# GregDMeyer/dynamite

Hardware: AMD Instinct MI355X
Metric: matrix-free H|psi> Gamplitudes/s, random-field Heisenberg (higher is better)
Workload: dtype f64 (complex128)

## Files before the change

### dynamite_amd/_lib.py

```python
import ctypes as C
import os

import numpy as np

from . import build as _build

_HERE = os.path.dirname(os.path.abspath(__file__))

i64p = C.POINTER(C.c_int64)
f64p = C.POINTER(C.c_double)
vp = C.c_void_p


class Subspace(C.Structure):
    _fields_ = [("type", C.c_int32), ("L", C.c_int64), ("space", C.c_int64), ("k", C.c_int64),
                ("ld_nchoosek", C.c_int64), ("nchoosek", i64p), ("dim", C.c_int64),
                ("state_map", i64p), ("rmap_indices", i64p), ("rmap_states", i64p), ("vec_swizzle", C.c_int32),
                ("site_perm", C.POINTER(C.c_int8))]


class Partition(C.Structure):
    _fields_ = [("rank", C.c_int32), ("nranks", C.c_int32)]


MULT_FN = C.CFUNCTYPE(C.c_int, vp, vp, vp)
REDUCE_FN = C.CFUNCTYPE(C.c_int, vp, f64p, C.c_int)


class Hooks(C.Structure):
    _fields_ = [("ctx", vp), ("mult", MULT_FN), ("allreduce_sum", REDUCE_FN),
                ("allreduce_max", REDUCE_FN)]


class SolverStats(C.Structure):
    _fields_ = [("reason", C.c_int32), ("its", C.c_int32), ("matvecs", C.c_int32),
                ("nconv", C.c_int32), ("err_est", C.c_double)]


MAXSEG, MAXBSEG, MAXR = 4, 8, 16


LP_COUNT = 9
LP_NAMES = ["tile_real_k0", "tile_real", "tile_cplx", "tile_kvar_real", "tile_kvar_cplx", "gather_real",
            "gather_kvar_real", "gather_cplx", "gather_kvar_cplx"]
LP_KVAR, LP_CPLX, LP_GATHER = (3, 4, 6, 8), (2, 4, 7, 8), (5, 6, 7, 8)


class DevQuad(C.Structure):
    _fields_ = [("mask_tile", C.c_uint32), ("mask_loc", C.c_uint32), ("src", C.c_uint32),
                ("nslots", C.c_uint32), ("sign_tile", C.c_uint32 * 4), ("sign_ext", C.c_uint64 * 4),
                ("coeff", C.c_double * 4)]


class DevPass(C.Structure):
    _fields_ = [("nseg", C.c_int32), ("seg_off", C.c_int32 * MAXSEG), ("seg_len", C.c_int32 * MAXSEG),
                ("seg_pos", C.c_int32 * MAXSEG), ("nbseg", C.c_int32), ("bseg_off", C.c_int32 * MAXBSEG),
                ("bseg_len", C.c_int32 * MAXBSEG), ("bseg_pos", C.c_int32 * MAXBSEG),
                ("sign_base", C.c_uint64), ("accumulate", C.c_int32), ("need_tile", C.c_int32),
                ("has_diag", C.c_int32), ("cache_policy", C.c_int32), ("dext_begin", C.c_uint32), ("dext_end", C.c_uint32),
                ("dbucket", C.c_uint32 * (MAXR + 1)), ("loop", C.c_uint32 * (LP_COUNT + 1)),
                ("nquads", C.c_int32), ("n_eff", C.c_int32), ("quads", vp), ("dot_out", vp), ("zinit", vp), ("zscale", C.c_double), ("zinit2", vp), ("z2re", C.c_double), ("z2im", C.c_double),
                ("tile_bits", C.c_int32), ("log_rows", C.c_int32),
                ("swz_shift", C.c_int32), ("swz_xor_y", C.c_uint32), ("swz_xor_src", C.c_uint32), ("block_offset", C.c_uint32),
                ("pos_tmask", C.c_uint32), ("dtile", vp), ("tabs", vp), ("tabvals", vp), ("tab_loop", C.c_uint32 * 3),
                ("pad_tab", C.c_uint32), ("gbucket", C.c_uint32 * (MAXR + 1)), ("pad_g", C.c_uint32)]


class DevTab(C.Structure):
    _fields_ = [("mask_tile", C.c_uint32), ("mask_loc", C.c_uint32), ("src", C.c_uint32), ("first", C.c_uint32),
                ("z_tile", C.c_uint32), ("flags", C.c_uint32), ("tpos", C.c_uint32), ("twid", C.c_uint32),
                ("epos", C.c_uint32), ("ewid", C.c_uint32), ("z_ext", C.c_uint64), ("ik", C.c_uint64),
                ("ksign", C.c_uint32), ("nbits", C.c_uint32)]


class Xfer(C.Structure):
    _fields_ = [("partner", C.c_int32), ("pass_id", C.c_int32), ("offset", C.c_int64), ("count", C.c_int64)]


MAT_DEFAULT, MAT_FORCE_GATHER, MAT_USE_GLDS, MAT_HOST_ONLY = 0, 1, 2, 4
MAT_REAL_PACKED = 16
EXCHANGE_AUTO, EXCHANGE_PARTNER, EXCHANGE_TRANSPOSE = 0, 1, 2
PHASE_ALL, PHASE_EXCHANGE, PHASE_COMPUTE = 0, 1, 2
MAT_AMIN_SHIFT = 8
WHICH = {"lowest": 0, "highest": 1, "exterior": 2, "target": 3}
CONVERGED_TOL, CONVERGED_ITS, DIVERGED_ITS, DIVERGED_BREAKDOWN, DIVERGED_SYMMETRY_LOST = 1, 2, -1, -2, -3

SIGNATURES = {
    "dnm_last_error": (C.c_char_p, []),
    "dnm_version": (C.c_int, []),
    "dnm_device_count": (C.c_int, [C.POINTER(C.c_int)]),
    "dnm_set_device": (C.c_int, [C.c_int]),
    "dnm_malloc": (C.c_int, [C.POINTER(vp), C.c_size_t]),
    "dnm_free": (C.c_int, [vp]),
    "dnm_memcpy_h2d": (C.c_int, [vp, vp, C.c_size_t, vp]),
    "dnm_memcpy_d2h": (C.c_int, [vp, vp, C.c_size_t, vp]),
    "dnm_stream_synchronize": (C.c_int, [vp]),
    "dnm_subspace_dim": (C.c_int, [C.POINTER(Subspace), i64p]),
    "dnm_idx_to_state": (C.c_int, [C.POINTER(Subspace), C.c_int64, i64p, i64p]),
    "dnm_state_to_idx": (C.c_int, [C.POINTER(Subspace), C.c_int64, i64p, i64p]),
    "dnm_mat_create": (C.c_int, [C.c_int64, i64p, i64p, i64p, f64p, C.POINTER(Subspace),
                                 C.POINTER(Subspace), C.c_int, C.c_int, C.POINTER(Partition),
                                 C.POINTER(vp)]),
    "dnm_check_conserves": (C.c_int, [C.c_int64, i64p, i64p, i64p, f64p, C.POINTER(Subspace),
                                      C.POINTER(Subspace), C.c_int, C.POINTER(C.c_int), vp]),
    "dnm_reduced_density_matrix": (C.c_int, [vp, C.POINTER(Subspace), C.c_int, i64p, vp, vp]),
    "dnm_vec_set_random_swz": (C.c_int, [vp, C.c_int64, C.c_uint64, C.c_int64, C.c_int, vp]),
    "dnm_vec_swizzle_copy": (C.c_int, [vp, vp, C.c_int64, C.c_int, vp]),
    "dnm_vec_unpack_real": (C.c_int, [vp, vp, C.c_int64, C.c_int, C.c_int, vp]),
    "dnm_vec_layout_unpack_real": (C.c_int, [C.POINTER(Subspace), C.POINTER(Partition), vp, vp, vp]),
    "dnm_vec_layout_size": (C.c_int, [C.POINTER(Subspace), C.POINTER(C.c_int64)]),
    "dnm_vec_layout_partition": (C.c_int, [C.POINTER(Subspace), C.c_int, C.c_int, i64p, i64p, i64p, i64p]),
    "dnm_vec_layout_blocks": (C.c_int, [C.POINTER(Subspace), C.c_int64, i64p, i64p, i64p]),
    "dnm_vec_layout_copy": (C.c_int, [C.POINTER(Subspace), C.POINTER(Partition), vp, vp, C.c_int, vp]),
    "dnm_vec_layout_copy_f64": (C.c_int, [C.POINTER(Subspace), C.POINTER(Partition), vp, vp, C.c_int, vp]),
    "dnm_vec_layout_zero_padding": (C.c_int, [C.POINTER(Subspace), C.POINTER(Partition), vp, vp]),
    "dnm_vec_layout_positions": (C.c_int, [C.POINTER(Subspace), C.POINTER(Partition), C.c_int64, vp, vp, vp]),
    "dnm_vec_layout_positions_host": (C.c_int, [C.POINTER(Subspace), C.POINTER(Partition), C.c_int64, i64p, i64p]),
    "dnm_vec_layout_set_random": (C.c_int, [C.POINTER(Subspace), C.POINTER(Partition), vp, C.c_uint64, vp]),
# ... 122 lines not shown
```

### dynamite_amd/csrc/mat.cpp

```cpp
#include "mat.h"
#include "vec_api.h"
#include "row_fused.h"

#include <algorithm>
#include <cstring>

namespace dnm {

static thread_local std::string g_err;

void set_error(const char *fmt, ...) {
  char buf[1024];
  va_list ap;
  va_start(ap, fmt);
  vsnprintf(buf, sizeof(buf), fmt, ap);
  va_end(ap);
  g_err = buf;
}

int DevBuf::alloc(size_t nbytes) {
  release();
  if (nbytes == 0) nbytes = 16;
  DNM_HIP(hipMalloc(&p, nbytes));
  bytes = nbytes;
// ... 377 lines not shown
            auto it = std::find_if(all.begin(), all.end(), [&](const auto &g) { return g.first == st; });
            if (it == all.end()) { all.push_back({st, {}}); it = all.end() - 1; }
            it->second.push_back(t);
          }
        std::stable_sort(all.begin(), all.end(), [](const auto &a, const auto &b) { return a.second.size() > b.second.size(); });
        for (auto &g : all)
          if (g.second.size() >= 3 && groups.size() < MAXDGROUPS) groups.push_back(std::move(g));
      }
      auto grouped = [&](uint32_t st) {
        return std::any_of(groups.begin(), groups.end(), [&](const auto &g) { return g.first == st; });
      };
      for (int j = 0; j < R; ++j) {
        lst.clear();
        for (const RowTerm &t : dm->terms) {
          uint32_t st = compress_to_tile(t.sign & tb, ps);
          if (st == 0 || (int)(st >> lognt) != j) continue;
          if (use_table && (t.sign & ~tb) == 0) {
            for (uint32_t tc = 0; tc < (1u << B); ++tc)
              out->h_dtile[tc] += (__builtin_popcount(tc & st) & 1) ? -t.coeff : t.coeff;
          } else if ((t.sign & ~tb) != 0 && grouped(st)) {
            continue;
          } else {
            lst.push_back(t);
          }
        }
        d.dbucket[j] = (uint32_t)quads.size();
        push_diag_list(lst);
      }
      for (int j = R; j <= MAXR; ++j) d.dbucket[j] = (uint32_t)quads.size();
      std::vector<std::pair<uint32_t, uint32_t>> where(groups.size());
      for (size_t g = 0; g < groups.size(); ++g) {
        std::vector<RowTerm> outside = groups[g].second;
        for (RowTerm &t : outside) t.sign &= ~tb;
        where[g].first = (uint32_t)quads.size();
        push_diag_list(outside);
        where[g].second = (uint32_t)quads.size() - where[g].first;
      }
      for (int j = 0; j < R; ++j) {
        d.gbucket[j] = (uint32_t)quads.size();
        for (size_t g = 0; g < groups.size(); ++g) {
          if ((int)(groups[g].first >> lognt) != j) continue;
          DevQuad q = empty_quad();
          q.sign_tile[0] = groups[g].first;
          q.mask_loc = where[g].first;
          q.src = where[g].second;
          q.nslots = 1;
          quads.push_back(q);
        }
      }
      for (int j = R; j <= MAXR; ++j) d.gbucket[j] = (uint32_t)quads.size();
    }
  }

  struct Rec { int loop; DevQuad q; };
  std::vector<Rec> recs;
  std::vector<DevTab> tabs_tile, tabs_gather;
  std::vector<double> tabvals;
  auto push_tabs = [&](const RowMask &m, uint64_t mloc, bool gather, int src) -> bool {
    std::vector<uint64_t> zs;
    if (!table_form(op, m, &zs)) return false;
    const int nb = __builtin_popcountll(m.mask);
    int pb[MAXTABBITS];
    for (int q = 0, pos = 0; pos < 64; ++pos)
      if ((m.mask >> pos) & 1ull) pb[q++] = pos;
    for (uint64_t z : zs) {
      DevTab T;
      memset(&T, 0, sizeof(T));
      T.mask_tile = compress_to_tile(mloc & tb, ps);
      T.mask_loc = (uint32_t)mloc;
      T.src = (uint32_t)src;
      T.nbits = (uint32_t)nb;
      const uint32_t zt = compress_to_tile(z & tb, ps);
      T.z_tile = zt & ((1u << lognt) - 1u);
      T.z_ext = z & ~tb;
      T.first = (uint32_t)(tabvals.size() / 2);
      for (int k = 0; k < R; ++k)
        if (__builtin_popcount((uint32_t)k & (zt >> lognt)) & 1) T.ksign |= 1u << k;
      for (int q = 0; q < nb; ++q) {
        if ((tb >> pb[q]) & 1ull) {
          const int tpos = __builtin_ctz(compress_to_tile((uint64_t)1 << pb[q], ps));
          if (tpos < lognt) {
            T.tpos |= (uint32_t)tpos << (8 * q);
            T.twid |= 1u << (8 * q);
          } else {
            T.flags |= 1u;
            for (int k = 0; k < R; ++k)
              if ((k >> (tpos - lognt)) & 1) T.ik |= (uint64_t)1 << (4 * k + q);
          }
        } else {
          T.epos |= (uint32_t)pb[q] << (8 * q);
          T.ewid |= 1u << (8 * q);
        }
      }
      for (int j = 0; j < (1 << nb); ++j) {
        uint64_t rowbits = 0;
        for (int q = 0; q < nb; ++q)
          if ((j >> q) & 1) rowbits |= (uint64_t)1 << pb[q];
        double re = 0.0, im = 0.0;
        for (const RowTerm &t : m.terms) {
          if ((t.sign & ~m.mask) != z) continue;
          const double c = (__builtin_popcountll(rowbits & t.sign & m.mask) & 1) ? -t.coeff : t.coeff;
          (t.is_imag ? im : re) += c;
        }
        tabvals.push_back(re);
        tabvals.push_back(im);
      }
      if (z == zs.back()) T.flags |= 2u;
      (gather ? tabs_gather : tabs_tile).push_back(T);
    }
    return true;
  };
  auto push_mask = [&](int idx, bool gather, int src) {
    const RowMask &m = op.masks[idx];
    const uint64_t mloc = m.mask & (((uint64_t)1 << n_eff) - 1);
    if (!gather) DNM_CHECK((mloc & ~tb) == 0, "internal: tile mask leaves the tile");
    if (push_tabs(m, mloc, gather, src)) return 0;
    std::vector<const RowTerm *> re, im;
    for (const RowTerm &t : m.terms) (t.is_imag ? im : re).push_back(&t);
    size_t ir = 0, ii = 0;
    while (ir < re.size() || ii < im.size()) {
      DevQuad q = empty_quad();
      q.mask_tile = compress_to_tile(mloc & tb, ps);
      q.mask_loc = (uint32_t)mloc;
      q.src = (uint32_t)src;
      q.nslots = m.pack_flip ? 1u : 0u;
      bool kvar = false, cplx = false;
      for (int s = 0; s < 2 && ir < re.size(); ++s, ++ir) {
        set_slot(q, s, *re[ir]);
        kvar |= (q.sign_tile[s] >> lognt) != 0;
      }
      for (int s = 2; s < 4 && ii < im.size(); ++s, ++ii) {
        set_slot(q, s, *im[ii]);
        kvar |= (q.sign_tile[s] >> lognt) != 0;
        cplx = true;
      }
      int loop;
      if (gather) loop = kvar ? (cplx ? LP_GATHER_KVAR_CPLX : LP_GATHER_KVAR_REAL) : (cplx ? LP_GATHER_CPLX : LP_GATHER_REAL);
      else if (kvar) loop = cplx ? LP_TILE_KVAR_CPLX : LP_TILE_KVAR_REAL;
      else if (cplx) loop = LP_TILE_CPLX;
      else loop = (q.mask_tile >> lognt) == 0 ? LP_TILE_REAL_K0 : LP_TILE_REAL;
      recs.push_back({loop, q});
    }
    return 0;
  };
  for (int idx : ps.tile_masks) DNM_TRY(push_mask(idx, false, 0));
  for (size_t i = 0; i < ps.gather_masks.size(); ++i)
    DNM_TRY(push_mask(ps.gather_masks[i], true, ps.gather_src[i]));
  for (int lp = 0; lp < LP_COUNT; ++lp) {
    d.loop[lp] = (uint32_t)quads.size();
    for (const Rec &r : recs) if (r.loop == lp) quads.push_back(r.q);
  }
  d.loop[LP_COUNT] = (uint32_t)quads.size();

  d.nquads = (int32_t)quads.size();
  d.need_tile = (d.has_diag || !ps.tile_masks.empty()) ? 1 : 0;
  d.tab_loop[0] = 0;
  d.tab_loop[1] = (uint32_t)tabs_tile.size();
  d.tab_loop[2] = (uint32_t)(tabs_tile.size() + tabs_gather.size());
  out->h_tabs = tabs_tile;
  out->h_tabs.insert(out->h_tabs.end(), tabs_gather.begin(), tabs_gather.end());
  out->h_tabvals = tabvals;
  d.tabs = nullptr;
  d.tabvals = nullptr;
  if (!out->h_tabs.empty() && !A.host_only) {
    DNM_TRY(out->tabs.upload(out->h_tabs.data(), out->h_tabs.size() * sizeof(DevTab)));
    DNM_TRY(out->tabvals.upload(out->h_tabvals.data(), out->h_tabvals.size() * sizeof(double)));
    d.tabs = (const DevTab *)out->tabs.p;
    d.tabvals = (const double *)out->tabvals.p;
  }
  out->h_quads = quads;
  if (!A.host_only) DNM_TRY(out->quads.upload(quads.data(), quads.size() * sizeof(DevQuad)));
  d.quads = (const DevQuad *)out->quads.p;
  d.dtile = nullptr;
  if (!out->h_dtile.empty() && !A.host_only) {
    DNM_TRY(out->dtile.upload(out->h_dtile.data(), out->h_dtile.size() * sizeof(double)));
    d.dtile = (const double *)out->dtile.p;
  }
  out->partner = ps.partner;
  out->n_eff = n_eff;
  out->y_off = ps.y_off;
  out->src_off = ps.src_off;
  return 0;
}

static hipStream_t S(void *stream) { return (hipStream_t)stream; }

static int launch_pass(const dnm_mat *A, const PassOnDevice &p, const DevPass &d, const void *x, void *y,
                       const void *xr, hipStream_t st, unsigned nparts = 1) {
  return launch_tile_pass(d, d.tile_bits, d.log_rows, (A->flags & DNM_MAT_USE_GLDS) != 0, p.n_eff, x, y, xr, st, nparts);
}

static size_t pass_dot_partials(const dnm_mat *, const PassOnDevice &p) {
  return (size_t)1 << (p.n_eff - p.desc.tile_bits);
}

}

using namespace dnm;

namespace dnm {
std::vector<ScMask> sc_masks(const std::vector<int64_t> &masks, const std::vector<int64_t> &mask_offsets,
                             const std::vector<int64_t> &signs, const std::vector<double> &rcoef, int L, bool xparity) {
  std::vector<ScMask> scm(masks.size());
// ... 1086 lines not shown
int dnm_mat_exchange_plan(const dnm_mat *A, int *nsend, dnm_xfer *sends, int *nrecv, dnm_xfer *recvs) {
  DNM_CHECK(A && nsend && nrecv, "null argument");
  *nsend = (int)A->plan.sends.size();
  *nrecv = (int)A->remote_passes.size();
  if (sends)
    for (size_t i = 0; i < A->plan.sends.size(); ++i)
      sends[i] = {A->plan.sends[i].partner, -1, A->plan.sends[i].offset, A->plan.sends[i].count};
  if (recvs)
    for (size_t i = 0; i < A->remote_passes.size(); ++i) {
      const auto &p = A->remote_passes[i];
      recvs[i] = {p->partner, (int32_t)i, p->src_off, (int64_t)1 << p->n_eff};
    }
  return 0;
}

int dnm_mat_mult_remote(dnm_mat *A, int32_t recv_index, const void *x_recv, void *y, void *stream) {
  DNM_CHECK(A && x_recv && y, "null argument");
  DNM_CHECK(!A->host_only, "host-only handle cannot multiply");
  DNM_CHECK(recv_index >= 0 && recv_index < (int)A->remote_passes.size(), "rank %d has no receive %d", A->rank,
            recv_index);
  const auto &p = A->remote_passes[recv_index];
  return launch_pass(A, *p, p->desc, x_recv, (char *)y + (size_t)p->y_off * 16, x_recv, S(stream));
}

int dnm_mat_norm_inf(dnm_mat *A, double *nrm, void *stream) {
  DNM_CHECK(A && nrm, "null argument");
  DNM_CHECK(!A->host_only, "host-only handle has no device tables");
  if (A->nrm != -1.0) {
    *nrm = A->nrm;
    return 0;
  }
  const int nb = norm_num_blocks(A->rows_local);
  DNM_TRY(A->scratch.alloc((size_t)nb * sizeof(double)));
  DNM_TRY(launch_norm(A->dmsc, A->left.dev, A->right.dev, A->rows_local, A->row0,
                      (double *)A->scratch.p, S(stream)));
  std::vector<double> h(nb);
  DNM_TRY(dnm_memcpy_d2h(h.data(), A->scratch.p, (size_t)nb * sizeof(double), stream));
  double best = 0.0;
  for (double v : h) best = std::max(best, v);
  if (A->nranks == 1) A->nrm = best;
  *nrm = best;
  return 0;
}

int dnm_mat_set_norm(dnm_mat *A, double nrm) {
  DNM_CHECK(A, "null matrix");
  A->nrm = nrm;
  return 0;
}

int dnm_mat_plan_describe(const dnm_mat *A, char *buf, size_t buflen) {
  DNM_CHECK(A && buf && buflen, "null argument");
  std::string s;
  if (A->hypercube) s = A->plan.describe(A->op);
  else if (A->use_sc3) {
    const Sc3Tab &T = A->sc3->ly->host;
    char tmp[512];
    if (A->sc3->tiled && A->sc3->graph)
      snprintf(tmp, sizeof tmp, "SpinConserve two-pass kernels on a bond graph, internal layout [T %d | W %d | Lo %d]: "
               "window pass (%zu workgroups, %d hops in LDS, %d gathered) then lo pass (%zu workgroups, %d hops in LDS, "
               "%d gathered), diagonal %s, coefficients %s\n", T.t, T.w, T.a, A->sc3->permB.size(), A->sc3->op.nldsB,
               A->sc3->op.ngatB, A->sc3->permA.size() / 8, A->sc3->op.nldsA, A->sc3->op.ngatA,
               A->sc3->diag_mode == 2 ? "on the fly" : (A->sc3->diag_mode == 1 ? "cached" : "none"),
               A->sc3->sym ? "real symmetric" : "complex");
    else if (A->sc3->tiled)
      snprintf(tmp, sizeof tmp, "SpinConserve two-pass kernels, internal layout [T %d | W %d | Lo %d]: window pass (%zu "
               "workgroups, %d bonds in LDS, %d gathered) then lo pass (%zu workgroups, %d bonds in LDS, %d gathered), "
               "diagonal %s, coefficients %s\n", T.t, T.w, T.a, A->sc3->permB.size(), T.w - 1,
               __builtin_popcountll(A->sc3->op.bondsB), A->sc3->permA.size() / 8, T.a - 1,
               __builtin_popcountll(A->sc3->op.bondsA),
               A->sc3->diag_mode == 2 ? "on the fly" : (A->sc3->diag_mode == 1 ? "cached" : "none"),
               A->sc3->sym ? "real symmetric" : "complex");
    else
      snprintf(tmp, sizeof tmp, "SpinConserve row kernel, internal layout [T %d | W %d | Lo %d] (positions by table)\n",
               T.t, T.w, T.a);
    s = tmp;
  } else if (A->sc_pair)
    s = A->scblock.lb ? "SpinConserve kernel, block form (" + std::to_string(A->scblock.lb) +
                            " low bits per workgroup in LDS, high bonds as block runs)\n"
                      : std::string("SpinConserve kernel (one row per thread, incremental colex rank)\n");
  else s = A->nranks > 1 ? "generic row-gather kernel (rows split in index order, columns through a window)\n"
                         : "generic row-gather kernel (non-hypercube subspace pair)\n";
  if (A->hypercube && !A->plan.use_tiled) s += "generic row-gather kernel in use\n";
  if (A->hypercube && A->plan.use_tiled) {
    size_t ntab = 0, nquad = 0;
    for (const auto &p : A->local_passes) { ntab += p->h_tabs.size(); nquad += p->desc.loop[LP_COUNT] - p->desc.loop[0]; }
    for (const auto &p : A->remote_passes) { ntab += p->h_tabs.size(); nquad += p->desc.loop[LP_COUNT] - p->desc.loop[0]; }
    if (ntab) s += "table records: " + std::to_string(ntab) + " (beside " + std::to_string(nquad) + " records of four terms)\n";
  }
  snprintf(buf, buflen, "%s", s.c_str());
  return 0;
}

int dnm_mat_export_pass(const dnm_mat *A, int remote, int idx, void *desc_out, size_t desc_bytes,
                        void *quads_out, size_t quad_bytes, int max_quads, int *nquads) {
  DNM_CHECK(A && nquads, "null argument");
  const auto &v = remote ? A->remote_passes : A->local_passes;
  DNM_CHECK(idx >= 0 && idx < (int)v.size(), "pass index out of range");
  const PassOnDevice &p = *v[idx];
  *nquads = (int)p.h_quads.size();
  if (desc_out) {
    DNM_CHECK(desc_bytes == sizeof(DevPass), "DevPass size mismatch (%zu vs %zu)", desc_bytes, sizeof(DevPass));
    memcpy(desc_out, &p.desc, sizeof(DevPass));
  }
  if (quads_out) {
    DNM_CHECK(quad_bytes == sizeof(DevQuad), "DevQuad size mismatch (%zu vs %zu)", quad_bytes, sizeof(DevQuad));
    DNM_CHECK(max_quads >= *nquads, "record buffer too small");
    if (!p.h_quads.empty()) memcpy(quads_out, p.h_quads.data(), p.h_quads.size() * sizeof(DevQuad));
// ... 60 lines not shown
```

### dynamite_amd/csrc/mat.h

```cpp
#pragma once

#include <memory>
#include <vector>

#include "kernels.h"
#include "plan.h"
#include "sc3.h"
#include "subspace.h"

namespace dnm {

struct DevBuf {
  void *p = nullptr;
  size_t bytes = 0;
  DevBuf() = default;
  DevBuf(const DevBuf &) = delete;
  DevBuf &operator=(const DevBuf &) = delete;
  ~DevBuf() { release(); }
  int alloc(size_t nbytes);
  int upload(const void *host, size_t nbytes);
  void release();
};

struct SubOwned {
  SubView host{};
  SubView dev{};
  std::vector<int64_t> nck, smap, rind, rstates, bucket;
  DevBuf d_nck, d_smap, d_rind, d_rstates, d_bucket;
  int init(const dnm_subspace *s, bool want_device);
};

struct PassOnDevice {
  DevPass desc{};
  std::vector<DevQuad> h_quads;
  DevBuf quads;
  std::vector<double> h_dtile;
  DevBuf dtile;
  std::vector<DevTab> h_tabs;
  std::vector<double> h_tabvals;
  DevBuf tabs, tabvals;
  int partner = -1;
  int n_eff = 0;
  int64_t y_off = 0, src_off = 0;
};

int rdm_release_scratch();

}

struct dnm_mat {
  std::vector<int64_t> masks, mask_offsets, signs;
  std::vector<double> real_coeffs;
  dnm::SubOwned left, right;
  int64_t M = 0, N = 0, m_local = 0, n_local = 0;
  int64_t row0 = 0;
  bool sc_pair = false;
  bool use_sc3 = false;
  std::unique_ptr<dnm::Sc3Mat> sc3;
  int64_t rows_local = 0;
  int64_t win_min = 0, win_max = -1;
  int rank = 0, nranks = 1;
  int flags = 0;
  bool xparity = false;
  bool host_only = false;

  bool hypercube = false;
  bool real_packed = false;
  dnm::OpForm op;
  dnm::Plan plan;
  std::vector<std::unique_ptr<dnm::PassOnDevice>> local_passes, remote_passes;

  dnm::DevBuf d_masks, d_offsets, d_signs, d_rcoeffs;
  dnm::DevMsc dmsc{};
  dnm::DevBuf d_pmasks, d_poffsets, d_psigns, d_prcoeffs;
  dnm::DevMsc dmsc_sc3{};
  dnm::DevBuf d_sclow;
  dnm::ScLow sclow{};
  dnm::DevBuf d_scblock;
  dnm::DevBuf d_scperm;
  dnm::ScBlock scblock{};
  bool row_fuse = true;
  int sc_nfast = 0;
  double expm_tstep = 0.0;
  int expm_m = 0;
  int expm_bound = 0;
  dnm::DevBuf d_scmasks;

  dnm_mat *tr_lo = nullptr, *tr_hi = nullptr;
  int tr_f = -1;
  ~dnm_mat();

  dnm::DevBuf diag;
  bool have_diag = false;
  double nrm = -1.0;
// ... 3 lines not shown
```

### dynamite_amd/csrc/matvec_kernels.hip

```cpp
#include <algorithm>
#include <cstdint>
#include <cstdlib>

#include "kernels.h"

namespace dnm {

typedef double2 c128;

#define GLOBAL_AS __attribute__((address_space(1)))
#define LDS_AS __attribute__((address_space(3)))

typedef double d2v __attribute__((ext_vector_type(2)));

typedef const __attribute__((address_space(4))) DevQuad CQuad;

__device__ __forceinline__ void store_through(c128 *p, double re, double im) {
  d2v v = {re, im};
  asm volatile("global_store_dwordx4 %0, %1, off sc1\n\ts_nop 1" ::"v"(p), "v"(v) : "memory");
}
__device__ __forceinline__ void store_streaming(c128 *p, double re, double im) {
  d2v v = {re, im};
  __builtin_nontemporal_store(v, reinterpret_cast<d2v *>(p));
}
// ... 105 lines not shown
      ar[k] = fma(cre, xv[k].x, ar[k]);
      ai[k] = fma(cre, xv[k].y, ai[k]);
      if constexpr (CPLX) {
        const double cim = flip_sign(a2, (uint32_t)__popc(k & s2) & 1u) + flip_sign(a3, (uint32_t)__popc(k & s3) & 1u);
        ar[k] = fma(-cim, xv[k].y, ar[k]);
        ai[k] = fma(cim, xv[k].x, ai[k]);
      }
    }
  }
}

template <int R, int LOGNT, bool KVAR, bool CPLX, bool GATHER, bool K0, bool PACK = false>
__device__ __forceinline__ void apply_records(CQuad *__restrict__ quads, uint32_t b, uint32_t e,
                                              double (&ar)[R], double (&ai)[R], const c128 *tile,
                                              const RowAddr<R> &RA, const c128 *__restrict__ x,
                                              const c128 *__restrict__ xr, uint32_t tid, uint64_t sbase,
                                              uint32_t skw = 0, uint32_t xrx = 0) {
  constexpr uint32_t NT = 1u << LOGNT;
  for (uint32_t qi = b; qi < e; ++qi) {
    CQuad &Q = quads[qi];
    const double a0 = slot_amp(Q, 0, tid, sbase);
    const double a1 = slot_amp(Q, 1, tid, sbase);
    double a2 = 0.0, a3 = 0.0;
    if constexpr (CPLX) {
      a2 = slot_amp(Q, 2, tid, sbase);
      a3 = slot_amp(Q, 3, tid, sbase);
    }
    c128 xv[R];
    if constexpr (GATHER) {
      const bool live = KVAR || (a0 + a1 != 0.0) || (CPLX && (a2 + a3 != 0.0));
      if (!__any(live)) continue;
      const c128 *__restrict__ src = Q.src ? xr : x;
      const uint32_t mloc = Q.mask_loc;
      const uint32_t xm = (skw ? (mloc ^ (((mloc >> skw) & ((1u << (skw - 4)) - 1u)) << 4)) : mloc) ^ (Q.src ? xrx : 0u);
      if (live) {
#pragma unroll
        for (int k = 0; k < R; ++k) xv[k] = *RA.at(src, k, xm);
      } else {
#pragma unroll
        for (int k = 0; k < R; ++k) xv[k] = make_double2(0.0, 0.0);
      }
    } else if constexpr (K0) {
      const c128 *p = tile + (tid ^ Q.mask_tile);
#pragma unroll
      for (int k = 0; k < R; ++k) xv[k] = p[k * NT];
    } else {
      const uint32_t mt = Q.mask_tile;
      const uint32_t p_lo = tid ^ (mt & (NT - 1u));
      const uint32_t mk = mt >> LOGNT;
#pragma unroll
      for (int k = 0; k < R; ++k) xv[k] = tile[p_lo + (((uint32_t)k ^ mk) << LOGNT)];
    }
    accum_record<R, LOGNT, KVAR, CPLX, PACK>(Q, a0, a1, a2, a3, xv, ar, ai);
  }
}

typedef const __attribute__((address_space(4))) DevTab CTab;

constexpr uint32_t TABB = 32;
constexpr uint32_t TABL_ENTRIES = TABB << MAXTABBITS;

template <int R, int LOGNT, bool GATHER>
__device__ __forceinline__ void apply_tabs(CTab *__restrict__ tabs, const c128 *__restrict__ vals, uint32_t b, uint32_t e,
                                           double (&ar)[R], double (&ai)[R], const c128 *tile, const RowAddr<R> &RA,
                                           const c128 *__restrict__ x, const c128 *__restrict__ xr, uint32_t tid,
                                           uint64_t sbase, uint32_t skw, uint32_t xrx, c128 *tabl) {
  constexpr uint32_t NT = 1u << LOGNT;
  c128 xv[R];
  bool fresh = true;
  for (uint32_t b0 = b; b0 < e; b0 += TABB) {
  const uint32_t b1 = (b0 + TABB < e) ? b0 + TABB : e;
  const uint32_t f0 = tabs[b0].first, f1 = tabs[b1 - 1].first + (1u << tabs[b1 - 1].nbits);
  __syncthreads();
  for (uint32_t i = tid; i < f1 - f0; i += NT) tabl[i] = vals[f0 + i];
  __syncthreads();
  for (uint32_t qi = b0; qi < b1; ++qi) {
    CTab &T = tabs[qi];
    if (fresh) {
      if constexpr (GATHER) {
        const c128 *__restrict__ src = T.src ? xr : x;
        const uint32_t mloc = T.mask_loc;
        const uint32_t xm = (skw ? (mloc ^ (((mloc >> skw) & ((1u << (skw - 4)) - 1u)) << 4)) : mloc) ^ (T.src ? xrx : 0u);
#pragma unroll
        for (int k = 0; k < R; ++k) xv[k] = *RA.at(src, k, xm);
      } else {
        const uint32_t mt = T.mask_tile;
        const uint32_t p_lo = tid ^ (mt & (NT - 1u));
        const uint32_t mk = mt >> LOGNT;
#pragma unroll
        for (int k = 0; k < R; ++k) xv[k] = tile[p_lo + (((uint32_t)k ^ mk) << LOGNT)];
      }
    }
    const uint32_t tp = T.tpos, tw = T.twid, ep = T.epos, ew = T.ewid;
    uint32_t it = 0, is = 0;
#pragma unroll
    for (int q = 0; q < MAXTABBITS; ++q) {
      it |= __builtin_amdgcn_ubfe(tid, (tp >> (8 * q)) & 0xffu, (tw >> (8 * q)) & 0xffu) << q;
      is |= ((uint32_t)(sbase >> ((ep >> (8 * q)) & 0xffu)) & ((ew >> (8 * q)) & 0xffu)) << q;
    }
    it |= is;
    const c128 *tv = tabl + (T.first - f0);
    const uint32_t psign = ((uint32_t)(__popc(tid & T.z_tile) + __popcll(sbase & T.z_ext)) & 1u) << 31;
    const uint32_t ks = T.ksign;
    const uint64_t ikp = T.ik;
    if (T.flags & 1u) {
#pragma unroll
// ... 99 lines not shown
      for (int k = 0; k < R; ++k) v[k] = *RA.at(x, k, 0u);
    }
#pragma unroll
    for (int k = 0; k < R; ++k) tile[tid + k * NT] = v[k];
  }
  DNM_PH(1, 1);

  double ar[R], ai[R];
  const bool late_y = P.accumulate && (P.cache_policy & 128);
  if (P.accumulate && !late_y) {
    if (P.cache_policy & 2) {
#pragma unroll
      for (int k = 0; k < R; ++k) {
        c128 v = load_streaming(RA.at((const c128 *)y, k, yx));
        ar[k] = v.x;
        ai[k] = v.y;
      }
    } else {
#pragma unroll
      for (int k = 0; k < R; ++k) {
        c128 v = *RA.at((const c128 *)y, k, yx);
        ar[k] = v.x;
        ai[k] = v.y;
      }
    }
  } else if (P.zinit) {
    const c128 *__restrict__ z = (const c128 *)P.zinit;
    const double zs = -P.zscale;
#pragma unroll
    for (int k = 0; k < R; ++k) {
      const c128 v = load_streaming(RA.at(z, k, yx));
      ar[k] = zs * v.x;
      ai[k] = zs * v.y;
    }
    if (P.zinit2) {
      const c128 *__restrict__ z2 = (const c128 *)P.zinit2;
      const double cr = P.z2re, ci = P.z2im;
#pragma unroll
      for (int k = 0; k < R; ++k) {
        const c128 v = load_streaming(RA.at(z2, k, yx));
        ar[k] = fma(cr, v.x, ar[k]);
        ar[k] = fma(-ci, v.y, ar[k]);
        ai[k] = fma(cr, v.y, ai[k]);
        ai[k] = fma(ci, v.x, ai[k]);
      }
    }
  } else {
#pragma unroll
    for (int k = 0; k < R; ++k) ar[k] = ai[k] = 0.0;
  }

  CQuad *__restrict__ quads = (CQuad *)P.quads;

#define DNM_LOOP(LP, KV, CX, GA, KZ) \
  apply_records<R, LOGNT, KV, CX, GA, KZ, PACK>(quads, P.loop[LP], P.loop[LP + 1], ar, ai, tile, RA, x, xr, tid, sbase, skw, P.swz_xor_src)
  if constexpr (GV >= 1) {
    DNM_LOOP(LP_GATHER_REAL, false, false, true, false);
    DNM_LOOP(LP_GATHER_KVAR_REAL, true, false, true, false);
    DNM_LOOP(LP_GATHER_CPLX, false, true, true, false);
    DNM_LOOP(LP_GATHER_KVAR_CPLX, true, true, true, false);
  }
#undef DNM_LOOP
  c128 *tabl = nullptr;
  if constexpr (TAB) {
    __shared__ __attribute__((aligned(16))) unsigned char tabl_mem[TABL_ENTRIES * 16];
    tabl = reinterpret_cast<c128 *>(tabl_mem);
  }
  if constexpr (TAB)
    apply_tabs<R, LOGNT, true>((CTab *)P.tabs, (const c128 *)P.tabvals, P.tab_loop[1], P.tab_loop[2], ar, ai, tile, RA, x, xr,
                               tid, sbase, skw, P.swz_xor_src, tabl);
  DNM_PH(2, 1);

  double dext = 0.0;
  if (P.has_diag) {
    const uint32_t lane = tid & 63u;
    const uint32_t nterm = (P.dext_end - P.dext_begin) * 4u;
    for (uint32_t t0 = 0; t0 < nterm; t0 += 64u) {
      const uint32_t t = t0 + lane;
      double v = 0.0;
      if (t < nterm) {
        CQuad &Q = quads[P.dext_begin + (t >> 2)];
        const uint32_t j = t & 3u;
        const uint32_t p = (uint32_t)__popcll(sbase & Q.sign_ext[j]) & 1u;
        v = flip_sign(Q.coeff[j], p);
      }
      dext += v;
    }
#pragma unroll
    for (int off = 32; off > 0; off >>= 1) dext += __shfl_xor(dext, off, 64);
  }
  double *cg = nullptr;
  if constexpr (TAB) {
    __shared__ double cg_mem[MAXDGROUPS];
    cg = cg_mem;
    if (P.has_diag) {
      const uint32_t lane = tid & 63u, g0 = P.gbucket[0], g1 = P.gbucket[R];
      for (uint32_t g = g0 + (tid >> 6); g < g1; g += (NT >> 6)) {
        const uint32_t q0 = quads[g].mask_loc, nterm = quads[g].src * 4u;
        double v = 0.0;
        for (uint32_t t0 = 0; t0 < nterm; t0 += 64u) {
          const uint32_t t = t0 + lane;
          if (t < nterm) {
            CQuad &Q = quads[q0 + (t >> 2)];
            const uint32_t j = t & 3u;
            v += flip_sign(Q.coeff[j], (uint32_t)__popcll(sbase & Q.sign_ext[j]) & 1u);
          }
        }
#pragma unroll
        for (int off = 32; off > 0; off >>= 1) v += __shfl_xor(v, off, 64);
        if (lane == 0) cg[g - g0] = v;
      }
    }
  }
  auto diag_part2 = [&]() {
  if (P.has_diag) {
// ... 2 lines not shown
    for (int j = 0; j < R; ++j) D[j] = 0.0;
    D[0] = dext;
    double dtab[R];
    if (P.dtile) {
#pragma unroll
      for (int k = 0; k < R; ++k) dtab[k] = P.dtile[tid + k * NT];
    }
#pragma unroll
    for (int j = 0; j < R; ++j)
      for (uint32_t q = P.dbucket[j]; q < P.dbucket[j + 1]; ++q) {
        const uint32_t ns = quads[q].nslots;
        double v = slot_amp(quads[q], 0, tid, sbase);
        if (ns > 1) v += slot_amp(quads[q], 1, tid, sbase);
        if (ns > 2) v += slot_amp(quads[q], 2, tid, sbase);
        if (ns > 3) v += slot_amp(quads[q], 3, tid, sbase);
        D[j] += v;
      }
    if constexpr (TAB) {
      const uint32_t g0 = P.gbucket[0];
#pragma unroll
      for (int j = 0; j < R; ++j)
        for (uint32_t q = P.gbucket[j]; q < P.gbucket[j + 1]; ++q)
          D[j] += flip_sign(cg[q - g0], (uint32_t)__popc(tid & quads[q].sign_tile[0]) & 1u);
    }
#pragma unroll
    for (int h = 1; h < R; h <<= 1) {
#pragma unroll
      for (int i = 0; i < R; ++i) {
        if ((i & h) == 0) {
          double a = D[i], b = D[i | h];
          D[i] = a + b;
          D[i | h] = a - b;
        }
      }
    }
    if (P.dtile) {
#pragma unroll
      for (int k = 0; k < R; ++k) D[k] += dtab[k];
    }
#pragma unroll
    for (int k = 0; k < R; ++k) {
      c128 xs = tile[tid + k * NT];
      ar[k] = fma(D[k], xs.x, ar[k]);
      ai[k] = fma(D[k], xs.y, ai[k]);
    }
  }
  };
  __syncthreads();
  DNM_PRIO_LDS();
  DNM_PH(3, 0);
  diag_part2();

  DNM_PH(4, 0);
#define DNM_LOOP(LP, KV, CX, GA, KZ) \
  apply_records<R, LOGNT, KV, CX, GA, KZ, PACK>(quads, P.loop[LP], P.loop[LP + 1], ar, ai, tile, RA, x, xr, tid, sbase, skw, P.swz_xor_src)
  DNM_LOOP(LP_TILE_REAL_K0, false, false, false, true);
  DNM_LOOP(LP_TILE_REAL, false, false, false, false);
  DNM_LOOP(LP_TILE_CPLX, false, true, false, false);
  DNM_LOOP(LP_TILE_KVAR_REAL, true, false, false, false);
  DNM_LOOP(LP_TILE_KVAR_CPLX, true, true, false, false);
  if constexpr (GV == 0) {
    DNM_LOOP(LP_GATHER_REAL, false, false, true, false);
    DNM_LOOP(LP_GATHER_KVAR_REAL, true, false, true, false);
    DNM_LOOP(LP_GATHER_CPLX, false, true, true, false);
    DNM_LOOP(LP_GATHER_KVAR_CPLX, true, true, true, false);
  }
#undef DNM_LOOP
  if constexpr (TAB)
    apply_tabs<R, LOGNT, false>((CTab *)P.tabs, (const c128 *)P.tabvals, P.tab_loop[0], P.tab_loop[1], ar, ai, tile, RA, x, xr,
                                tid, sbase, skw, P.swz_xor_src, tabl);

  DNM_PH(5, 0);
  DNM_PRIO_MEM();
  if (late_y) {
    c128 w[R];
#pragma unroll
    for (int k = 0; k < R; ++k) w[k] = load_streaming(RA.at((const c128 *)y, k, yx));
#pragma unroll
    for (int k = 0; k < R; ++k) {
      ar[k] += w[k].x;
      ai[k] += w[k].y;
    }
  }
  DNM_PH(6, 1);
  if (P.cache_policy & 64) {
#pragma unroll
    for (int k = 0; k < R; ++k) store_streaming(RA.at(y, k, yx), ar[k], ai[k]);
  } else if (P.cache_policy & 1) {
#pragma unroll
    for (int k = 0; k < R; ++k) store_through(RA.at(y, k, yx), ar[k], ai[k]);
  } else {
#pragma unroll
    for (int k = 0; k < R; ++k) *RA.at(y, k, yx) = make_double2(ar[k], ai[k]);
  }

  DNM_PH(7, 1);
  if (P.dot_out) {
    double dr = 0.0, di = 0.0, dn = 0.0;
#pragma unroll
    for (int k = 0; k < R; ++k) {
      const c128 xs = tile[tid + k * NT];
      dr = fma(xs.x, ar[k], dr);
      dr = fma(xs.y, ai[k], dr);
      di = fma(xs.x, ai[k], di);
      di = fma(-xs.y, ar[k], di);
      dn = fma(ar[k], ar[k], dn);
      dn = fma(ai[k], ai[k], dn);
    }
#pragma unroll
    for (int off = 32; off > 0; off >>= 1) {
      dr += __shfl_xor(dr, off, 64);
      di += __shfl_xor(di, off, 64);
      dn += __shfl_xor(dn, off, 64);
    }
    __shared__ double dred[3 * (NT / 64 > 0 ? NT / 64 : 1)];
    if ((tid & 63u) == 0) {
      dred[3 * (tid >> 6)] = dr;
      dred[3 * (tid >> 6) + 1] = di;
      dred[3 * (tid >> 6) + 2] = dn;
    }
// ... 926 lines not shown
```

### dynamite_amd/csrc/plan.h

```cpp
#pragma once

#include <cstdint>
#include <string>
#include <vector>

#include "dnm_common.h"

namespace dnm {

constexpr int MAXSEG = 4;
constexpr int MAXBSEG = 8;
constexpr int MAXSRC = 8;
constexpr int MAXR = 16;

struct RowTerm {
  uint64_t sign;
  double coeff;
  int is_imag;
};

struct RowMask {
  uint64_t mask;
  std::vector<RowTerm> terms;
  bool zero_mask_offdiag = false;
  bool pack_flip = false;
};

struct OpForm {
  bool packed = false;
  int n = 0;
  std::vector<RowMask> masks;
};

struct DevQuad {
  uint32_t mask_tile;
  uint32_t mask_loc;
  uint32_t src;
  uint32_t nslots;
  uint32_t sign_tile[4];
  uint64_t sign_ext[4];
  double coeff[4];
};

constexpr int MAXTABBITS = 4;
struct DevTab {
  uint32_t mask_tile;
  uint32_t mask_loc;
  uint32_t src;
  uint32_t first;
  uint32_t z_tile;
  uint32_t flags;
  uint32_t tpos, twid;
  uint32_t epos, ewid;
  uint64_t z_ext;
  uint64_t ik;
  uint32_t ksign;
  uint32_t nbits;
};

enum {
  LP_TILE_REAL_K0 = 0,
  LP_TILE_REAL,
  LP_TILE_CPLX,
  LP_TILE_KVAR_REAL,
  LP_TILE_KVAR_CPLX,
  LP_GATHER_REAL,
  LP_GATHER_KVAR_REAL,
  LP_GATHER_CPLX,
  LP_GATHER_KVAR_CPLX,
  LP_COUNT
};

struct DevPass {
  int32_t nseg;
  int32_t seg_off[MAXSEG], seg_len[MAXSEG], seg_pos[MAXSEG];
  int32_t nbseg;
  int32_t bseg_off[MAXBSEG], bseg_len[MAXBSEG], bseg_pos[MAXBSEG];
  uint64_t sign_base;
  int32_t accumulate;
  int32_t need_tile;
  int32_t has_diag;
  int32_t cache_policy;
  uint32_t dext_begin, dext_end;
  uint32_t dbucket[MAXR + 1];
  uint32_t loop[LP_COUNT + 1];
  int32_t nquads;
  int32_t n_eff;
  const DevQuad *quads;
  double *dot_out;
  const void *zinit;
  double zscale;
  const void *zinit2;
  double z2re, z2im;
  int32_t tile_bits;
  int32_t log_rows;
  int32_t swz_shift;
  uint32_t swz_xor_y, swz_xor_src;
  uint32_t block_offset;
  uint32_t pos_tmask;
  const double *dtile;
  const DevTab *tabs;
  const double *tabvals;
  uint32_t tab_loop[3];
  uint32_t pad_tab;
  uint32_t gbucket[MAXR + 1];
  uint32_t pad_g;
};
constexpr uint32_t MAXDGROUPS = 64;

struct PassSpec {
  int B = 0;
  int logR = 0;
  int nseg = 0;
  int seg_len[MAXSEG] = {0}, seg_pos[MAXSEG] = {0};
  std::vector<int> tile_masks;
  std::vector<int> gather_masks;
  std::vector<int> gather_src;
  bool has_diag = false;
  bool accumulate = false;
  int partner = -1;
  int n_eff = 0;
  int64_t y_off = 0, src_off = 0;
  uint64_t sign_extra = 0;
  int glen = 0, gpos = 0;
  uint64_t tile_bits() const {
    uint64_t m = 0;
    for (int j = 0; j < nseg; ++j) m |= (((uint64_t)1 << seg_len[j]) - 1) << seg_pos[j];
    return m;
  }
};

struct PlanConfig {
  int B = 12;
  int logR = -1;
  int amin = -1;
  int mode = 2;
  int gbits = -1;
  int Bw = 0, logRw = 0;
  int window_first = -1;
  int gbits_window = -1;
  int cache_policy = 226;
  int max_gather_span = 0;
  int diag_last = -1;
  int swz = 0;
};

struct Plan {
  int n = 0, n_loc = 0;
  int rank = 0, nranks = 1;
  PlanConfig cfg;
  std::vector<PassSpec> local;
  std::vector<PassSpec> remote;
  struct Send { int partner; int64_t offset, count; };
  std::vector<Send> sends;
  bool use_tiled = false;
  std::string describe(const OpForm &op) const;
};

PlanConfig plan_config_from_env();
// ... 4 lines not shown
```

Baseline: 64.27.

## Add exchange-record form exploiting XX+YY sign structure in Heisenberg hopping terms

Real records holding two terms with equal or opposite coefficients are rewritten into an exchange form. A single parity test on a wave-uniform row index then decides which of the R rows are live, so dead rows skip their loads and the kernel does one FMA per live row instead of evaluating two signed amplitudes. These records are split into dedicated sub-ranges (xloop) per loop class and processed by a new apply_exchange routine when no table or gather-bucket records exist. This aims to cut arithmetic and tile/global loads for flip-flop terms, at the cost of extra per-record branching, more kernel code, and a wave-uniform assumption on the lane bits of the sign mask.

```diff
diff --git a/dynamite_amd/_lib.py b/dynamite_amd/_lib.py
--- a/dynamite_amd/_lib.py
+++ b/dynamite_amd/_lib.py
@@ -44,6 +44,8 @@
 LP_NAMES = ["tile_real_k0", "tile_real", "tile_cplx", "tile_kvar_real", "tile_kvar_cplx", "gather_real",
             "gather_kvar_real", "gather_cplx", "gather_kvar_cplx"]
 LP_KVAR, LP_CPLX, LP_GATHER = (3, 4, 6, 8), (2, 4, 7, 8), (5, 6, 7, 8)
+XL_COUNT = 5
+XL_OF_LOOP = {0: 0, 1: 1, 3: 2, 5: 3, 6: 4}
 
 
 class DevQuad(C.Structure):
@@ -63,7 +65,8 @@
                 ("tile_bits", C.c_int32), ("log_rows", C.c_int32),
                 ("swz_shift", C.c_int32), ("swz_xor_y", C.c_uint32), ("swz_xor_src", C.c_uint32), ("block_offset", C.c_uint32),
                 ("pos_tmask", C.c_uint32), ("dtile", vp), ("tabs", vp), ("tabvals", vp), ("tab_loop", C.c_uint32 * 3),
-                ("pad_tab", C.c_uint32), ("gbucket", C.c_uint32 * (MAXR + 1)), ("pad_g", C.c_uint32)]
+                ("pad_tab", C.c_uint32), ("gbucket", C.c_uint32 * (MAXR + 1)), ("pad_g", C.c_uint32),
+                ("xloop", C.c_uint32 * XL_COUNT), ("pad_x", C.c_uint32)]
 
 
 class DevTab(C.Structure):
diff --git a/dynamite_amd/csrc/mat.cpp b/dynamite_amd/csrc/mat.cpp
--- a/dynamite_amd/csrc/mat.cpp
+++ b/dynamite_amd/csrc/mat.cpp
@@ -453,8 +453,35 @@
     }
   }
 
-  struct Rec { int loop; DevQuad q; };
+  struct Rec { int loop; DevQuad q; bool xc; };
   std::vector<Rec> recs;
+  const bool xc_on = []() { const char *e = knob("DNM_EXCHANGE_RECORDS"); return !(e && e[0] == '0'); }() && !op.packed;
+  auto exchange_form = [&](DevQuad &q) -> bool {
+    const double c0 = q.coeff[0], c1 = q.coeff[1];
+    if (c0 == 0.0 || (c1 != c0 && c1 != -c0)) return false;
+    const int w0 = __builtin_popcount(q.sign_tile[0]) + __builtin_popcountll(q.sign_ext[0]);
+    const int w1 = __builtin_popcount(q.sign_tile[1]) + __builtin_popcountll(q.sign_ext[1]);
+    if (w1 < w0) {
+      std::swap(q.sign_tile[0], q.sign_tile[1]);
+      std::swap(q.sign_ext[0], q.sign_ext[1]);
+      std::swap(q.coeff[0], q.coeff[1]);
+    }
+    const uint32_t zt = q.sign_tile[0] ^ q.sign_tile[1];
+    const uint64_t ze = q.sign_ext[0] ^ q.sign_ext[1];
+    const uint32_t lanes = (1u << std::min(6, lognt)) - 1u;
+    if ((zt == 0 && ze == 0) || (zt & lanes) != 0) return false;
+    uint32_t kz = 0;
+    uint64_t ks = 0;
+    for (int k = 0; k < R; ++k) {
+      if (__builtin_popcount((uint32_t)k & (zt >> lognt)) & 1) kz |= 1u << k;
+      if (__builtin_popcount((uint32_t)k & (q.sign_tile[0] >> lognt)) & 1) ks |= (uint64_t)1 << k;
+    }
+    q.sign_tile[2] = zt;
+    q.sign_ext[2] = ze;
+    q.sign_tile[3] = (c1 == c0 ? 0u : 1u) | (kz << 16);
+    q.sign_ext[3] = ks;
+    return true;
+  };
   std::vector<DevTab> tabs_tile, tabs_gather;
   std::vector<double> tabvals;
   auto push_tabs = [&](const RowMask &m, uint64_t mloc, bool gather, int src) -> bool {
@@ -526,7 +553,8 @@
       q.src = (uint32_t)src;
       q.nslots = m.pack_flip ? 1u : 0u;
       bool kvar = false, cplx = false;
-      for (int s = 0; s < 2 && ir < re.size(); ++s, ++ir) {
+      int nre = 0;
+      for (int s = 0; s < 2 && ir < re.size(); ++s, ++ir, ++nre) {
         set_slot(q, s, *re[ir]);
         kvar |= (q.sign_tile[s] >> lognt) != 0;
       }
@@ -540,16 +568,23 @@
       else if (kvar) loop = cplx ? LP_TILE_KVAR_CPLX : LP_TILE_KVAR_REAL;
       else if (cplx) loop = LP_TILE_CPLX;
       else loop = (q.mask_tile >> lognt) == 0 ? LP_TILE_REAL_K0 : LP_TILE_REAL;
-      recs.push_back({loop, q});
+      const bool xc = xc_on && !cplx && nre == 2 && exchange_form(q);
+      recs.push_back({loop, q, xc});
     }
     return 0;
   };
   for (int idx : ps.tile_masks) DNM_TRY(push_mask(idx, false, 0));
   for (size_t i = 0; i < ps.gather_masks.size(); ++i)
     DNM_TRY(push_mask(ps.gather_masks[i], true, ps.gather_src[i]));
+  const bool xc_pass = tabs_tile.empty() && tabs_gather.empty() && d.gbucket[MAXR] == d.gbucket[0];
+  out->n_exchange = 0;
   for (int lp = 0; lp < LP_COUNT; ++lp) {
     d.loop[lp] = (uint32_t)quads.size();
-    for (const Rec &r : recs) if (r.loop == lp) quads.push_back(r.q);
+    const bool split = xc_pass && XL_OF_LOOP[lp] >= 0;
+    for (const Rec &r : recs) if (r.loop == lp && !(split && r.xc)) quads.push_back(r.q);
+    if (XL_OF_LOOP[lp] >= 0) d.xloop[XL_OF_LOOP[lp]] = (uint32_t)quads.size();
+    if (!split) continue;
+    for (const Rec &r : recs) if (r.loop == lp && r.xc) { quads.push_back(r.q); ++out->n_exchange; }
   }
   d.loop[LP_COUNT] = (uint32_t)quads.size();
 
@@ -1742,8 +1777,25 @@
 int dnm_mat_plan_describe(const dnm_mat *A, char *buf, size_t buflen) {
   DNM_CHECK(A && buf && buflen, "null argument");
   std::string s;
-  if (A->hypercube) s = A->plan.describe(A->op);
-  else if (A->use_sc3) {
+  if (A->hypercube) {
+    s = A->plan.describe(A->op);
+    std::string t;
+    size_t line = 0, pos = 0;
+    while (pos < s.size()) {
+      size_t nl = s.find('\n', pos);
+      if (nl == std::string::npos) nl = s.size();
+      t.append(s, pos, nl - pos);
+      const size_t nloc_p = A->local_passes.size(), ip = line - 1;
+      if (line >= 1 && A->plan.use_tiled && ip < nloc_p + A->remote_passes.size()) {
+        const int nx = ip < nloc_p ? A->local_passes[ip]->n_exchange : A->remote_passes[ip - nloc_p]->n_exchange;
+        if (nx) t += " exchange_records=" + std::to_string(nx);
+      }
+      t += '\n';
+      pos = nl + 1;
+      ++line;
+    }
+    s = t;
+  } else if (A->use_sc3) {
     const Sc3Tab &T = A->sc3->ly->host;
     char tmp[512];
     if (A->sc3->tiled && A->sc3->graph)
diff --git a/dynamite_amd/csrc/mat.h b/dynamite_amd/csrc/mat.h
--- a/dynamite_amd/csrc/mat.h
+++ b/dynamite_amd/csrc/mat.h
@@ -40,6 +40,7 @@
   std::vector<double> h_tabvals;
   DevBuf tabs, tabvals;
   int partner = -1;
+  int n_exchange = 0;
   int n_eff = 0;
   int64_t y_off = 0, src_off = 0;
 };
diff --git a/dynamite_amd/csrc/matvec_kernels.hip b/dynamite_amd/csrc/matvec_kernels.hip
--- a/dynamite_amd/csrc/matvec_kernels.hip
+++ b/dynamite_amd/csrc/matvec_kernels.hip
@@ -181,6 +181,60 @@
       for (int k = 0; k < R; ++k) xv[k] = tile[p_lo + (((uint32_t)k ^ mk) << LOGNT)];
     }
     accum_record<R, LOGNT, KVAR, CPLX, PACK>(Q, a0, a1, a2, a3, xv, ar, ai);
+  }
+}
+
+template <int R, int LOGNT, bool GATHER, bool K0>
+__device__ __forceinline__ void apply_exchange(CQuad *__restrict__ quads, uint32_t b, uint32_t e,
+                                               double (&ar)[R], double (&ai)[R], const c128 *tile,
+                                               const RowAddr<R> &RA, const c128 *__restrict__ x,
+                                               const c128 *__restrict__ xr, uint32_t tid, uint32_t wv, uint64_t sbase,
+                                               uint32_t skw, uint32_t xrx) {
+  constexpr uint32_t NT = 1u << LOGNT;
+  constexpr uint32_t ALL = (1u << R) - 1u;
+  for (uint32_t qi = b; qi < e; ++qi) {
+    CQuad &Q = quads[qi];
+    const uint32_t f = Q.sign_tile[3];
+    const uint32_t dead0 = ((uint32_t)(__popc(wv & Q.sign_tile[2]) + __popcll(sbase & Q.sign_ext[2])) ^ f) & 1u;
+    const uint32_t live = K0 ? (dead0 ? 0u : ALL) : ((dead0 ? (f >> 16) : ~(f >> 16)) & ALL);
+    if (live == 0u) continue;
+    const double a0 = slot_amp(Q, 0, tid, sbase);
+    const double cth = a0 + a0;
+    c128 xv[R];
+    if constexpr (K0) {
+      const c128 *p = tile + (tid ^ Q.mask_tile);
+#pragma unroll
+      for (int k = 0; k < R; ++k) xv[k] = p[k * NT];
+#pragma unroll
+      for (int k = 0; k < R; ++k) {
+        ar[k] = fma(cth, xv[k].x, ar[k]);
+        ai[k] = fma(cth, xv[k].y, ai[k]);
+      }
+    } else {
+      if constexpr (GATHER) {
+        const c128 *__restrict__ src = Q.src ? xr : x;
+        const uint32_t mloc = Q.mask_loc;
+        const uint32_t xm = (skw ? (mloc ^ (((mloc >> skw) & ((1u << (skw - 4)) - 1u)) << 4)) : mloc) ^ (Q.src ? xrx : 0u);
+#pragma unroll
+        for (int k = 0; k < R; ++k)
+          if ((live >> k) & 1u) xv[k] = *RA.at(src, k, xm);
+      } else {
+        const uint32_t mt = Q.mask_tile;
+        const uint32_t p_lo = tid ^ (mt & (NT - 1u));
+        const uint32_t mk = mt >> LOGNT;
+#pragma unroll
+        for (int k = 0; k < R; ++k)
+          if ((live >> k) & 1u) xv[k] = tile[p_lo + (((uint32_t)k ^ mk) << LOGNT)];
+      }
+      const uint32_t ks = (uint32_t)Q.sign_ext[3];
+#pragma unroll
+      for (int k = 0; k < R; ++k)
+        if ((live >> k) & 1u) {
+          const double c = flip_sign(cth, (ks >> k) & 1u);
+          ar[k] = fma(c, xv[k].x, ar[k]);
+          ai[k] = fma(c, xv[k].y, ai[k]);
+        }
+    }
   }
 }
 
@@ -386,15 +440,24 @@
 
   CQuad *__restrict__ quads = (CQuad *)P.quads;
 
+  constexpr bool XC = !PACK && !TAB;
+  const uint32_t wv = (uint32_t)__builtin_amdgcn_readfirstlane((int)tid);
 #define DNM_LOOP(LP, KV, CX, GA, KZ) \
   apply_records<R, LOGNT, KV, CX, GA, KZ, PACK>(quads, P.loop[LP], P.loop[LP + 1], ar, ai, tile, RA, x, xr, tid, sbase, skw, P.swz_xor_src)
+#define DNM_LOOP_X(LP, XL, KV, GA, KZ)                                                                                          \
+  do {                                                                                                                          \
+    apply_records<R, LOGNT, KV, false, GA, KZ, PACK>(quads, P.loop[LP], XC ? P.xloop[XL] : P.loop[LP + 1], ar, ai, tile, RA, x, \
+                                                     xr, tid, sbase, skw, P.swz_xor_src);                                       \
+    if constexpr (XC)                                                                                                           \
+      apply_exchange<R, LOGNT, GA, KZ>(quads, P.xloop[XL], P.loop[LP + 1], ar, ai, tile, RA, x, xr, tid, wv, sbase, skw,        \
+                                       P.swz_xor_src);                                                                          \
+  } while (0)
   if constexpr (GV >= 1) {
-    DNM_LOOP(LP_GATHER_REAL, false, false, true, false);
-    DNM_LOOP(LP_GATHER_KVAR_REAL, true, false, true, false);
+    DNM_LOOP_X(LP_GATHER_REAL, XL_GATHER_REAL, false, true, false);
+    DNM_LOOP_X(LP_GATHER_KVAR_REAL, XL_GATHER_KVAR_REAL, true, true, false);
     DNM_LOOP(LP_GATHER_CPLX, false, true, true, false);
     DNM_LOOP(LP_GATHER_KVAR_CPLX, true, true, true, false);
   }
-#undef DNM_LOOP
   c128 *tabl = nullptr;
   if constexpr (TAB) {
     __shared__ __attribute__((aligned(16))) unsigned char tabl_mem[TABL_ENTRIES * 16];
@@ -503,20 +566,19 @@
   diag_part2();
 
   DNM_PH(4, 0);
-#define DNM_LOOP(LP, KV, CX, GA, KZ) \
-  apply_records<R, LOGNT, KV, CX, GA, KZ, PACK>(quads, P.loop[LP], P.loop[LP + 1], ar, ai, tile, RA, x, xr, tid, sbase, skw, P.swz_xor_src)
-  DNM_LOOP(LP_TILE_REAL_K0, false, false, false, true);
-  DNM_LOOP(LP_TILE_REAL, false, false, false, false);
+  DNM_LOOP_X(LP_TILE_REAL_K0, XL_TILE_K0, false, false, true);
+  DNM_LOOP_X(LP_TILE_REAL, XL_TILE_REAL, false, false, false);
   DNM_LOOP(LP_TILE_CPLX, false, true, false, false);
-  DNM_LOOP(LP_TILE_KVAR_REAL, true, false, false, false);
+  DNM_LOOP_X(LP_TILE_KVAR_REAL, XL_TILE_KVAR_REAL, true, false, false);
   DNM_LOOP(LP_TILE_KVAR_CPLX, true, true, false, false);
   if constexpr (GV == 0) {
-    DNM_LOOP(LP_GATHER_REAL, false, false, true, false);
-    DNM_LOOP(LP_GATHER_KVAR_REAL, true, false, true, false);
+    DNM_LOOP_X(LP_GATHER_REAL, XL_GATHER_REAL, false, true, false);
+    DNM_LOOP_X(LP_GATHER_KVAR_REAL, XL_GATHER_KVAR_REAL, true, true, false);
     DNM_LOOP(LP_GATHER_CPLX, false, true, true, false);
     DNM_LOOP(LP_GATHER_KVAR_CPLX, true, true, true, false);
   }
 #undef DNM_LOOP
+#undef DNM_LOOP_X
   if constexpr (TAB)
     apply_tabs<R, LOGNT, false>((CTab *)P.tabs, (const c128 *)P.tabvals, P.tab_loop[0], P.tab_loop[1], ar, ai, tile, RA, x, xr,
                                 tid, sbase, skw, P.swz_xor_src, tabl);
diff --git a/dynamite_amd/csrc/plan.h b/dynamite_amd/csrc/plan.h
--- a/dynamite_amd/csrc/plan.h
+++ b/dynamite_amd/csrc/plan.h
@@ -71,6 +71,17 @@
   LP_COUNT
 };
 
+enum {
+  XL_TILE_K0 = 0,
+  XL_TILE_REAL,
+  XL_TILE_KVAR_REAL,
+  XL_GATHER_REAL,
+  XL_GATHER_KVAR_REAL,
+  XL_COUNT
+};
+constexpr int XL_OF_LOOP[LP_COUNT] = {XL_TILE_K0, XL_TILE_REAL, -1, XL_TILE_KVAR_REAL, -1, XL_GATHER_REAL,
+                                      XL_GATHER_KVAR_REAL, -1, -1};
+
 struct DevPass {
   int32_t nseg;
   int32_t seg_off[MAXSEG], seg_len[MAXSEG], seg_pos[MAXSEG];
@@ -105,6 +116,8 @@
   uint32_t pad_tab;
   uint32_t gbucket[MAXR + 1];
   uint32_t pad_g;
+  uint32_t xloop[XL_COUNT];
+  uint32_t pad_x;
 };
 constexpr uint32_t MAXDGROUPS = 64;
 
```

Result: slower. 61.03 (-5.0%).
